# AlwinEsch/pvr.rtl.radiofm

Measured on AMD Instinct MI355X. Metric: IQ MS/s demodulated (whole node) + achieved HBM GB/s on FIR stage, higher is better.
Workload: dtype f32

## Files before the change

### pvr.rtl.radiofm_amd/csrc/fmd_k_resample.hip.h

```cpp
#pragma once

#include "fmd_k_common.hip.h"

namespace fmd
{

__global__ void k_rs_table(const float* __restrict__ coeff, unsigned order, float p, float pstep,
                           unsigned A, float* __restrict__ ktab, unsigned row_stride, unsigned margin,
                           int* __restrict__ pidx)
{
  const unsigned i = blockIdx.x;
  if (i >= A)
    return;
  const float pf = p + (float)i * pstep;
  const int pi = (int)pf;
  const float k1 = pf - (float)pi;
  const float k0 = 1 - k1;
  for (unsigned j = threadIdx.x; j <= order; j += blockDim.x)
    ktab[(size_t)i * row_stride + margin + j] = coeff[j] * k0 + coeff[j + 1] * k1;
  if (threadIdx.x == 0)
    pidx[i] = pi;
}

#ifndef FMD_RS_R
#define FMD_RS_R 6
#endif
#ifndef FMD_RS_B
#define FMD_RS_B 8
#endif
constexpr int RS_R = FMD_RS_R;
constexpr int RS_B = FMD_RS_B;
inline unsigned rs_table_margin(float step)
{
  return unsigned(RS_B + (RS_R - 1) * (int(step) + 2) + 7) / 8 * 8;
}

__global__ __launch_bounds__(256) void k_resample(const float2* __restrict__ br, unsigned Hbb,
                                                  unsigned order, const float* __restrict__ ktab,
                                                  unsigned row_stride, unsigned margin,
                                                  const int* __restrict__ pidx, unsigned A,
                                                  float2* __restrict__ out, unsigned Hout, unsigned C,
                                                  unsigned CP)
{
  const unsigned c = blockIdx.x * 64 + threadIdx.x;
  const unsigned wy = (unsigned)__builtin_amdgcn_readfirstlane((int)threadIdx.y);
  const unsigned i0 = (blockIdx.y * blockDim.y + wy) * RS_R;
  if (i0 >= A)
    return;
  const int nr = (int)min((unsigned)RS_R, A - i0);
  int off[RS_R];
  const float* kp[RS_R];
  const int top = pidx[i0 + nr - 1];
#pragma unroll
  for (int r = 0; r < RS_R; r++)
  {
    const int rr = r < nr ? r : nr - 1;
    off[r] = top - pidx[i0 + rr];
    kp[r] = ktab + (size_t)(i0 + rr) * row_stride + margin - off[r];
  }
  float2 acc[RS_R];
#pragma unroll
  for (int r = 0; r < RS_R; r++)
    acc[r] = make_float2(0.0f, 0.0f);
  const char* __restrict__ rp = reinterpret_cast<const char*>(br + (size_t)(Hbb + (unsigned)top) * CP);
  const unsigned lane_off = c * (unsigned)sizeof(float2);
  const size_t row_bytes = (size_t)CP * sizeof(float2);
  const int off0 = off[0];
  const int tend = off0 + (int)order;

  float2 xn[RS_B];
#pragma unroll
  for (int q = 0; q < RS_B; q++)
  {
    xn[q] = *reinterpret_cast<const float2*>(rp + lane_off);
    rp -= row_bytes;
  }
  for (int t = 0; t <= tend; t += RS_B)
  {
    float2 xs[RS_B];
#pragma unroll
    for (int q = 0; q < RS_B; q++)
      xs[q] = xn[q];
#pragma unroll
    for (int q = 0; q < RS_B; q++)
    {
      xn[q] = *reinterpret_cast<const float2*>(rp + lane_off);
      rp -= row_bytes;
    }
    float kk[RS_R][RS_B];
#pragma unroll
    for (int r = 0; r < RS_R; r++)
    {
#pragma unroll
      for (int q = 0; q < RS_B; q++)
        kk[r][q] = kp[r][t + q];
    }
    bool literal = false;
    if (!(t >= off0 && t + RS_B - 1 <= (int)order))
    {
      bool fin = true;
#pragma unroll
      for (int q = 0; q < RS_B; q++)
        fin = fin && __builtin_isfinite(xs[q].x) && __builtin_isfinite(xs[q].y);
      literal = FMD_ANY_LANE(!fin);
    }
    if (!literal)
    {
#pragma unroll
      for (int q = 0; q < RS_B; q++)
      {
#pragma unroll
        for (int r = 0; r < RS_R; r++)
        {
          acc[r].x += kk[r][q] * xs[q].x;
          acc[r].y += kk[r][q] * xs[q].y;
        }
      }
    }
    else
    {
#pragma unroll
      for (int q = 0; q < RS_B; q++)
      {
#pragma unroll
        for (int r = 0; r < RS_R; r++)
        {
          const int j = t + q - off[r];
          if (j >= 0 && j <= (int)order)
          {
            acc[r].x += kk[r][q] * xs[q].x;
            acc[r].y += kk[r][q] * xs[q].y;
          }
        }
      }
    }
  }
  if (c < C)
  {
#pragma unroll
    for (int r = 0; r < RS_R; r++)
      if (r < nr)
        out[(size_t)(Hout + i0 + r) * CP + c] = make_float2(acc[r].y, acc[r].x);
  }
}


constexpr int RSR_ROWS = 96;
constexpr int RSR_HEAD = 4 + 4;

template <int R, bool FMA = false>
__device__ __forceinline__ void rs_walk_asm(fmd_f2v (&acc)[R], unsigned& off, unsigned& cnt, unsigned lane16,
                                            unsigned wrap, unsigned klo, unsigned khi, unsigned kinc);
template <>
__device__ __forceinline__ void rs_walk_asm<4, false>(fmd_f2v (&acc)[4], unsigned& off, unsigned& cnt,
                                                      unsigned lane16, unsigned wrap, unsigned klo, unsigned khi,
                                                      unsigned kinc)
{
#include "fmd_rs_walk_r4.inc"
}
template <>
__device__ __forceinline__ void rs_walk_asm<2, false>(fmd_f2v (&acc)[2], unsigned& off, unsigned& cnt,
                                                      unsigned lane16, unsigned wrap, unsigned klo, unsigned khi,
                                                      unsigned kinc)
{
#include "fmd_rs_walk_r2.inc"
}
template <>
__device__ __forceinline__ void rs_walk_asm<2, true>(fmd_f2v (&acc)[2], unsigned& off, unsigned& cnt,
                                                     unsigned lane16, unsigned wrap, unsigned klo, unsigned khi,
                                                     unsigned kinc)
{
#include "fmd_rs_walk_r2_fma.inc"
}

template <int R, int NW>
__device__ __forceinline__ void rs_warm_asm(unsigned tlo, unsigned thi, unsigned gstride, unsigned rounds,
                                            unsigned pace);
template <>
__device__ __forceinline__ void rs_warm_asm<4, 4>(unsigned tlo, unsigned thi, unsigned gstride, unsigned rounds,
                                                  unsigned pace)
{
#include "fmd_rs_warm_r4w4.inc"
}
template <>
__device__ __forceinline__ void rs_warm_asm<2, 8>(unsigned tlo, unsigned thi, unsigned gstride, unsigned rounds,
                                                  unsigned pace)
{
#include "fmd_rs_warm_r2w8.inc"
}
template <>
__device__ __forceinline__ void rs_warm_asm<2, 4>(unsigned tlo, unsigned thi, unsigned gstride, unsigned rounds,
                                                  unsigned pace)
{
#include "fmd_rs_warm_r2w4.inc"
}

template <int R, int RSR_NW>
__global__ __launch_bounds__(64) void k_rs_plan(const float* __restrict__ coeff, unsigned order, float p,
                                                float pstep, unsigned A, int RB, unsigned NBR,
                                                float* __restrict__ tab, unsigned nbm,
                                                int* __restrict__ head, int* __restrict__ steptab)
{
  const unsigned g = blockIdx.x;
  auto pidx_of = [&](unsigned i) { return (int)(p + (float)i * pstep); };
  auto extent = [&](unsigned gg, int& top, int& nb) {
    const unsigned i0 = gg * R;
    if (i0 >= A)
    {
      top = 0;
      nb = 0;
      return;
    }
    const unsigned il = min(i0 + R - 1, A - 1);
    top = (pidx_of(il) + RB) >> 3;
    const int bot = (pidx_of(i0) - (int)order + RB) >> 3;
    nb = top - bot + 1;
    nb += nb & 1;
  };
  int top, nb;
  extent(g, top, nb);
  float k0[R], k1[R];
  int pi[R];
#pragma unroll
  for (int r = 0; r < R; r++)
  {
    const unsigned i = min(g * R + r, A - 1);
    const float pf = p + (float)i * pstep;
    pi[r] = (int)pf;
    k1[r] = pf - (float)pi[r];
    k0[r] = 1 - k1[r];
  }
  for (int idx = threadIdx.x; idx < nb * 8 * R; idx += 64)
  {
    const int b = idx / (8 * R), q = (idx / R) & 7, r = idx % R;
    const int row = (top - b) * 8 + 7 - q - RB;
    float v = 0.0f;
#pragma unroll
    for (int rr = 0; rr < R; rr++)
      if (rr == r)
      {
        const int j = pi[rr] - row;
        if (j >= 0 && j <= (int)order)
          v = coeff[j] * k0[rr] + coeff[j + 1] * k1[rr];
      }
    tab[((size_t)g * nbm + b) * (8 * R) + (idx % (8 * R))] = v;
  }
  if (threadIdx.x == 0)
  {
    int* h = head + (size_t)g * RSR_HEAD;
    h[0] = top;
    h[1] = nb;
    h[2] = (int)(((unsigned)top % NBR) * 4096u);
    h[3] = 0;
#pragma unroll
    for (int r = 0; r < R; r++)
      h[4 + r] = pi[r];
    if (g % RSR_NW == 0)
    {
      int stop = 0, sbot = 0x7fffffff;
      for (unsigned w = 0; w < (unsigned)RSR_NW; w++)
      {
        int t, n;
        extent(g + w, t, n);
        if (n > 0)
        {
          stop = t;
          sbot = min(sbot, t - n + 1);
        }
      }
      steptab[2 * (g / RSR_NW)] = stop;
      steptab[2 * (g / RSR_NW) + 1] = sbot;
    }
  }
}

template <int R, int RSR_NW, bool FMA = false>
__global__ __launch_bounds__(64 * (RSR_NW + 1)) void k_resample_ring(
    const float2* __restrict__ br, unsigned Hbb, int RB, unsigned order, const float* __restrict__ tab,
    unsigned nbm, const int* __restrict__ head, const int* __restrict__ steptab, unsigned nsteps,
    unsigned steps_per_wg, unsigned NBR, unsigned A, float2* __restrict__ out, unsigned Hout, unsigned C,
    unsigned CP, unsigned prio)
{
  constexpr int RSR_PRE = RSR_ROWS / RSR_NW;
  constexpr int LEAD = 3;
  extern __shared__ __align__(16) unsigned char rsr_smem[];
  __shared__ unsigned nonfinite_s;
  const unsigned lane = threadIdx.x;
  const unsigned w = (unsigned)__builtin_amdgcn_readfirstlane((int)threadIdx.y);
  wave_prio(prio);
  const unsigned units = (CP / 64u) * nsteps;
  unsigned u0 = min(units, blockIdx.x * steps_per_wg);
  const unsigned u1 = min(units, u0 + steps_per_wg);
  if (u0 >= u1)
    return;
  unsigned c = 0, s0 = 0, s1 = 0, lane_off = 0;
  bool live = false;
  const unsigned ring_pairs = NBR * 4;
  const char* const gbase = reinterpret_cast<const char*>(br + ((ptrdiff_t)Hbb - (ptrdiff_t)RB) * (ptrdiff_t)CP);
  const size_t row_bytes = (size_t)CP * sizeof(float2);
  unsigned emax = 0u;
  auto look = [&](float2 v) {
    emax = max(emax, max(__float_as_uint(v.x) & 0x7fffffffu, __float_as_uint(v.y) & 0x7fffffffu));
  };
  auto ring_addr = [&](unsigned pair_slot, unsigned odd) {
    return reinterpret_cast<float2*>(rsr_smem + (size_t)pair_slot * 1024 + lane * 16 + odd * 8);
  };
  float2 pre[RSR_PRE];
  auto fetch = [&](int r0, int mine) {
    const char* rp = gbase + (size_t)(r0 + (int)w) * row_bytes;
#pragma unroll
    for (int n = 0; n < RSR_PRE; n++)
      if (n < mine)
      {
        const fmd_f2v v = __builtin_nontemporal_load(reinterpret_cast<const fmd_f2v*>(rp + lane_off));
        pre[n] = make_float2(v.x, v.y);
        rp += RSR_NW * row_bytes;
      }
  };
  auto stash = [&](int r0, int mine) {
    unsigned ps = ((unsigned)(r0 + (int)w) >> 1) % ring_pairs;
#pragma unroll
    for (int n = 0; n < RSR_PRE; n++)
      if (n < mine)
      {
        look(pre[n]);
        *ring_addr(ps, w & 1u) = pre[n];
        ps += RSR_NW / 2;
        ps = ps >= ring_pairs ? ps - ring_pairs : ps;
      }
    if (emax >= 0x7f800000u && live)
      nonfinite_s = 1u;
  };
  auto share = [&](int n_rows) { return (n_rows - (int)w + RSR_NW - 1) / RSR_NW; };
  const bool warmer = w == (unsigned)RSR_NW;
  auto warm = [&](unsigned step, int b0, int rounds) {
    if (rounds <= 0)
      return;
    const uint64_t ta = reinterpret_cast<uint64_t>(tab) + ((uint64_t)step * RSR_NW * nbm + (uint64_t)b0) * (32 * R);
    rs_warm_asm<R, RSR_NW>((unsigned)ta, (unsigned)(ta >> 32), nbm * (32u * R), (unsigned)rounds, 0u);
  };
  {
    const size_t gsz = (size_t)nbm * (8 * R) * sizeof(float);
    const char* t0 = reinterpret_cast<const char*>(tab);
    const size_t bytes = (size_t)nsteps * RSR_NW * gsz;
    const unsigned nx = (gridDim.x + 7u) / 8u, part = blockIdx.x / 8u;
    const size_t per = ((bytes + nx - 1) / nx + 15) & ~(size_t)15;
    const size_t lo = min(bytes, part * per), hi = min(bytes, lo + per);
    unsigned sink = 0;
    for (size_t o = lo + (size_t)(threadIdx.y * 64 + lane) * 16; o + 16 <= hi; o += (size_t)(RSR_NW + 1) * 64 * 16)
    {
      const uint4 v = *reinterpret_cast<const uint4*>(t0 + o);
      sink |= v.x ^ v.y ^ v.z ^ v.w;
    }
    if (sink == 0x7fc12345u)
      nonfinite_s = sink;
  }
  for (; u0 < u1; u0 += s1 - s0)
  {
  const unsigned grp = u0 / nsteps;
  s0 = u0 - grp * nsteps;
  s1 = min(nsteps, s0 + (u1 - u0));
  c = grp * 64 + lane;
  lane_off = c * (unsigned)sizeof(float2);
  live = c < C;
  emax = 0u;
  __syncthreads();
  if (threadIdx.x == 0 && threadIdx.y == 0)
    nonfinite_s = 0u;
  __syncthreads();
  int topb = steptab[2 * s0];
  {
    const int r_hi = topb * 8 + 7;
    for (int r0 = steptab[2 * s0 + 1] * 8; r0 <= r_hi; r0 += RSR_NW * RSR_PRE)
    {
      const int mine = warmer ? 0 : share(min(r_hi + 1 - r0, RSR_NW * RSR_PRE));
      fetch(r0, mine);
      stash(r0, mine);
    }
    if (warmer)
      warm(s0, 0, LEAD);
  }
  __syncthreads();
  for (unsigned s = s0; s < s1; s++)
  {
    const int ntop = s + 1 < s1 ? steptab[2 * (s + 1)] : topb;
    const int r_new0 = topb * 8 + 8;
    const int mine = warmer ? 0 : share((ntop - topb) * 8);
    fetch(r_new0, mine);
    if (warmer)
    {
      warm(s, LEAD, (int)nbm - 1 - LEAD);
      if (s + 1 < s1)
        warm(s + 1, 0, LEAD);
      lds_barrier();
      topb = ntop;
      lds_barrier();
      continue;
    }
    const unsigned g = s * RSR_NW + w;
    const int* __restrict__ h = head + (size_t)g * RSR_HEAD;
    const int gtop = h[0], nb = h[1];
    fmd_f2v acc[R];
#pragma unroll
    for (int r = 0; r < R; r++)
      acc[r] = fmd_f2v{0.0f, 0.0f};
    if (nb > 0)
    {
      const float* __restrict__ kp = tab + (size_t)g * nbm * (8 * R);
      if (__builtin_expect(nonfinite_s == 0u, 1))
      {
        unsigned off = (unsigned)h[2], cnt = (unsigned)nb >> 1;
        const uint64_t ka = reinterpret_cast<uint64_t>(kp);
        rs_walk_asm<R, FMA>(acc, off, cnt, (unsigned)(size_t)rsr_smem + lane * 16u, (NBR - 1u) * 4096u, (unsigned)ka,
                       (unsigned)(ka >> 32), 32u * R);
      }
      else
      {
        for (int b = 0; b < nb; b++)
        {
          const unsigned slot = (unsigned)(gtop - b) % NBR;
#pragma unroll
          for (int q = 0; q < 8; q++)
          {
            const int rowb = 7 - q;
            const float2 x = *ring_addr(slot * 4 + (unsigned)(rowb >> 1), (unsigned)rowb & 1u);
            const int row = (gtop - b) * 8 + rowb - RB;
#pragma unroll
            for (int r = 0; r < R; r++)
            {
              const int j = h[4 + r] - row;
              if (j >= 0 && j <= (int)order)
              {
                const float k = kp[(size_t)b * (8 * R) + q * R + r];
                if (FMA)
                {
                  acc[r].x = __builtin_fmaf(k, x.x, acc[r].x);
                  acc[r].y = __builtin_fmaf(k, x.y, acc[r].y);
                }
                else
                {
                  acc[r].x += k * x.x;
                  acc[r].y += k * x.y;
                }
              }
            }
          }
        }
      }
      if (live)
      {
#pragma unroll
        for (int r = 0; r < R; r++)
          if (g * R + r < A)
            out[(size_t)(Hout + g * R + r) * CP + c] = make_float2(acc[r].y, acc[r].x);
      }
    }
    lds_barrier();
    stash(r_new0, mine);
    topb = ntop;
    lds_barrier();
  }
  }
}

}
```

Measured before the change: 298,700.

## Prefetch per-step head records and unroll table warm-up loads in resampler

The table builder now stores, in each head record, the step-to-step delta of the top block. The ring kernel reads the whole record as one int4 and prefetches the next step's record a step ahead, so it no longer loads steptab and scattered head fields on the critical path. The nonfinite flag is read once into a scalar register before the branch. The L2 warm-up loop now keeps four 16-byte loads in flight and reduces them only at kernel exit, so the load latencies overlap. The cost is extra registers and a more complex header contract between the two kernels.

```diff
diff --git a/pvr.rtl.radiofm_amd/csrc/fmd_k_resample.hip.h b/pvr.rtl.radiofm_amd/csrc/fmd_k_resample.hip.h
--- a/pvr.rtl.radiofm_amd/csrc/fmd_k_resample.hip.h
+++ b/pvr.rtl.radiofm_amd/csrc/fmd_k_resample.hip.h
@@ -247,29 +247,36 @@
   }
   if (threadIdx.x == 0)
   {
-    int* h = head + (size_t)g * RSR_HEAD;
-    h[0] = top;
-    h[1] = nb;
-    h[2] = (int)(((unsigned)top % NBR) * 4096u);
-    h[3] = 0;
-#pragma unroll
-    for (int r = 0; r < R; r++)
-      h[4 + r] = pi[r];
-    if (g % RSR_NW == 0)
-    {
-      int stop = 0, sbot = 0x7fffffff;
+    auto step_extent = [&](unsigned s, int& stop, int& sbot) {
+      stop = 0;
+      sbot = 0x7fffffff;
       for (unsigned w = 0; w < (unsigned)RSR_NW; w++)
       {
         int t, n;
-        extent(g + w, t, n);
+        extent(s * RSR_NW + w, t, n);
         if (n > 0)
         {
           stop = t;
           sbot = min(sbot, t - n + 1);
         }
       }
-      steptab[2 * (g / RSR_NW)] = stop;
-      steptab[2 * (g / RSR_NW) + 1] = sbot;
+    };
+    const unsigned s = g / RSR_NW;
+    int stop, sbot, ntop, nbot;
+    step_extent(s, stop, sbot);
+    step_extent(s + 1, ntop, nbot);
+    int* h = head + (size_t)g * RSR_HEAD;
+    h[0] = top;
+    h[1] = nb;
+    h[2] = (int)(((unsigned)top % NBR) * 4096u);
+    h[3] = (s + 1) * (RSR_NW * R) < A ? ntop - stop : 0;
+#pragma unroll
+    for (int r = 0; r < R; r++)
+      h[4 + r] = pi[r];
+    if (g % RSR_NW == 0)
+    {
+      steptab[2 * s] = stop;
+      steptab[2 * s + 1] = sbot;
     }
   }
 }
@@ -339,21 +346,29 @@
     const uint64_t ta = reinterpret_cast<uint64_t>(tab) + ((uint64_t)step * RSR_NW * nbm + (uint64_t)b0) * (32 * R);
     rs_warm_asm<R, RSR_NW>((unsigned)ta, (unsigned)(ta >> 32), nbm * (32u * R), (unsigned)rounds, 0u);
   };
+  const unsigned wr = warmer ? 0u : w;
+  auto record = [&](unsigned step) {
+    return *reinterpret_cast<const int4*>(head + ((size_t)min(step, nsteps - 1u) * RSR_NW + wr) * RSR_HEAD);
+  };
+  uint4 warmed[4] = {};
+  unsigned sink = 0;
   {
     const size_t gsz = (size_t)nbm * (8 * R) * sizeof(float);
     const char* t0 = reinterpret_cast<const char*>(tab);
     const size_t bytes = (size_t)nsteps * RSR_NW * gsz;
-    const unsigned nx = (gridDim.x + 7u) / 8u, part = blockIdx.x / 8u;
+    const unsigned nx = (gridDim.x + 7u) / 8u, xpart = blockIdx.x / 8u;
     const size_t per = ((bytes + nx - 1) / nx + 15) & ~(size_t)15;
-    const size_t lo = min(bytes, part * per), hi = min(bytes, lo + per);
-    unsigned sink = 0;
-    for (size_t o = lo + (size_t)(threadIdx.y * 64 + lane) * 16; o + 16 <= hi; o += (size_t)(RSR_NW + 1) * 64 * 16)
-    {
-      const uint4 v = *reinterpret_cast<const uint4*>(t0 + o);
-      sink |= v.x ^ v.y ^ v.z ^ v.w;
-    }
-    if (sink == 0x7fc12345u)
-      nonfinite_s = sink;
+    const size_t lo = min(bytes, xpart * per), hi = min(bytes, lo + per);
+    constexpr size_t stride = (size_t)(RSR_NW + 1) * 64 * 16;
+    for (size_t o = lo + (size_t)(threadIdx.y * 64 + lane) * 16; o + 16 <= hi; o += 4 * stride)
+    {
+#pragma unroll
+      for (int k = 0; k < 4; k++)
+      {
+        sink |= warmed[k].x ^ warmed[k].y ^ warmed[k].z ^ warmed[k].w;
+        warmed[k] = *reinterpret_cast<const uint4*>(t0 + min(o + k * stride, hi - 16));
+      }
+    }
   }
   for (; u0 < u1; u0 += s1 - s0)
   {
@@ -369,6 +384,7 @@
     nonfinite_s = 0u;
   __syncthreads();
   int topb = steptab[2 * s0];
+  int4 cur = record(s0);
   {
     const int r_hi = topb * 8 + 7;
     for (int r0 = steptab[2 * s0 + 1] * 8; r0 <= r_hi; r0 += RSR_NW * RSR_PRE)
@@ -383,23 +399,30 @@
   __syncthreads();
   for (unsigned s = s0; s < s1; s++)
   {
-    const int ntop = s + 1 < s1 ? steptab[2 * (s + 1)] : topb;
+    const bool last = s + 1 == s1;
+    const int delta = last ? 0 : cur.w;
     const int r_new0 = topb * 8 + 8;
-    const int mine = warmer ? 0 : share((ntop - topb) * 8);
+    const int mine = warmer ? 0 : share(delta * 8);
     fetch(r_new0, mine);
+    unsigned flag = 0u, sn = s + 1;
+    if (!warmer)
+      flag = (unsigned)__builtin_amdgcn_readfirstlane((int)nonfinite_s);
+    asm volatile("" : "+s"(flag), "+s"(sn));
+    const int4 nxt = record(sn);
     if (warmer)
     {
       warm(s, LEAD, (int)nbm - 1 - LEAD);
-      if (s + 1 < s1)
+      if (!last)
         warm(s + 1, 0, LEAD);
       lds_barrier();
-      topb = ntop;
+      topb += delta;
+      cur = nxt;
       lds_barrier();
       continue;
     }
     const unsigned g = s * RSR_NW + w;
     const int* __restrict__ h = head + (size_t)g * RSR_HEAD;
-    const int gtop = h[0], nb = h[1];
+    const int gtop = cur.x, nb = cur.y;
     fmd_f2v acc[R];
 #pragma unroll
     for (int r = 0; r < R; r++)
@@ -407,9 +430,9 @@
     if (nb > 0)
     {
       const float* __restrict__ kp = tab + (size_t)g * nbm * (8 * R);
-      if (__builtin_expect(nonfinite_s == 0u, 1))
-      {
-        unsigned off = (unsigned)h[2], cnt = (unsigned)nb >> 1;
+      if (__builtin_expect(flag == 0u, 1))
+      {
+        unsigned off = (unsigned)cur.z, cnt = (unsigned)nb >> 1;
         const uint64_t ka = reinterpret_cast<uint64_t>(kp);
         rs_walk_asm<R, FMA>(acc, off, cnt, (unsigned)(size_t)rsr_smem + lane * 16u, (NBR - 1u) * 4096u, (unsigned)ka,
                        (unsigned)(ka >> 32), 32u * R);
@@ -457,10 +480,16 @@
     }
     lds_barrier();
     stash(r_new0, mine);
-    topb = ntop;
+    topb += delta;
+    cur = nxt;
     lds_barrier();
   }
   }
-}
-
-}
+#pragma unroll
+  for (int k = 0; k < 4; k++)
+    sink |= warmed[k].x ^ warmed[k].y ^ warmed[k].z ^ warmed[k].w;
+  if (sink == 0x7fc12345u)
+    nonfinite_s = sink;
+}
+
+}
```

New measurement: 300,300 (median of 6 runs). No clear change (+0.6%).
